# BananaFalls/LDPC-NeuralNetwork-Decoder

Measured on AMD Instinct MI355X. Metric: codewords/s at fixed SNR (BG2, 10 iters), higher is better.
Workload: dtype f32

## Files before the change

### ldpc-neuralnetwork-decoder_amd/csrc/flood.hip

```cpp
#include <algorithm>
#include <cstdio>
#include <cstdlib>
#include <string>
#include <vector>

#include "flood_host.hpp"

namespace ldpc {

__global__ void es_init_kernel(int32_t *ctl, uint64_t *staged, uint32_t *all_words) {
    const int t = threadIdx.x;
    if (t < 4) ctl[t] = 0;
    if (t < 4) staged[t] = 0;
    if (t < 64) all_words[t] = ~0u;
}

__global__ __launch_bounds__(1024) void counters_reduce_kernel(const uint32_t *__restrict__ partials, int64_t nwg,
                                                               uint64_t *counters, int32_t *batch_iters,
                                                               const int32_t *gate) {
    if (gate && *gate == 0) return;
    uint64_t acc[4] = {0, 0, 0, 0};
    uint32_t mx = 0;
    for (int64_t r = threadIdx.x; r < nwg; r += blockDim.x) {
        const uint32_t *row = partials + r * kPartRow;
// ... 63 lines not shown
        if (aw) {
            const int t = w * 32 + __builtin_ctz(aw);
            if (t < max_iter) { tstar = t; break; }
        }
    }
    const int wave = __builtin_amdgcn_readfirstlane(threadIdx.x >> 6);
    const Lane L = make_lane(T, nullptr, B);
    Ctx C;
    C.T = T;
    C.out_dtype = out_dtype;
    C.bits = bits;
    int errs = 0;
    emit_from_words(C, L, ws_words + ((int64_t)blockIdx.x * max_iter + tstar) * T.Nb, ~0ull, wave, errs);
    if (iters_out && L.valid && L.k == 0) iters_out[L.frame] = tstar + 1;
    const int nf = (int)min<int64_t>((int64_t)T.FG, B - (int64_t)blockIdx.x * T.FG);
    if (partials) reduce_counters(red, L, errs, tstar + 1, nf, T.Z, partials + (int64_t)blockIdx.x * kPartRow);
}

__global__ void fill_i32_kernel(int32_t *p, int32_t v) { *p = v; }

__global__ __launch_bounds__(256) void bp_math_kernel(const float *__restrict__ x, int64_t n,
                                                      float *__restrict__ th, float *__restrict__ at) {
    const int64_t i = (int64_t)blockIdx.x * blockDim.x + threadIdx.x;
    if (i >= n) return;
    const float v = x[i];
    if (th) th[i] = tanh_half(v);
    if (at) at[i] = two_atanh(v);
}

template <int ES>
__global__ __launch_bounds__(512) void flood_redo_kernel(FloodTables T, const float *__restrict__ llr, int64_t B,
// ... 71 lines not shown

bool has_redo(const ldpc_graph *g, int algo, int es) {
    return g->fixed_id != 0 && algo == LDPC_ALGO_MINSUM && (es == LDPC_ES_OFF || es == LDPC_ES_FRAME);
}

template <int ALGO, int ES>
int launch_flood(const ldpc_graph *g, const float *llr, int64_t B, int max_iter, float alpha, int out_dtype,
                 void *bits, const Outs &O, const EsWs &W, hipStream_t s, uint32_t *redo = nullptr) {
    const size_t lds = flood_lds_bytes(g, ES);
    const int64_t nwg = (B + g->FG - 1) / g->FG;
    if (g->fixed_id != 0) {
        const dim3 grid((unsigned)nwg), block(64 * g->ft.W);
        if constexpr (ALGO == LDPC_ALGO_MINSUM && (ES == LDPC_ES_OFF || ES == LDPC_ES_FRAME)) {
            if (redo) {
                LDPC_HIP(hipMemsetAsync(redo, 0, sizeof(uint32_t), s));
                int rc = launch_fixed_minsum(g->fixed_id, ES, grid, block, lds, s, g->ft, llr, B, max_iter, alpha,
                                             out_dtype, bits, O, W, redo);
                if (rc != LDPC_OK) return rc;
                auto again = flood_redo_kernel<ES>;
                LDPC_HIP(hipFuncSetAttribute(reinterpret_cast<const void *>(again),
                                             hipFuncAttributeMaxDynamicSharedMemorySize, (int)lds));
                Outs Or = O;
                Or.timeline = nullptr;
                hipLaunchKernelGGL(again, dim3((unsigned)std::min<int64_t>(nwg, kRedoGrid)), block, lds, s, g->ft, llr,
                                   B, max_iter, alpha, out_dtype, bits, Or, (const uint32_t *)redo);
                LDPC_CHECK_LAUNCH("flood_redo_kernel");
                return LDPC_OK;
            }
        }
        return ALGO == LDPC_ALGO_MINSUM
                   ? launch_fixed_minsum(g->fixed_id, ES, grid, block, lds, s, g->ft, llr, B, max_iter, alpha,
                                         out_dtype, bits, O, W, nullptr)
                   : launch_fixed_bp(g->fixed_id, ES, grid, block, lds, s, g->ft, llr, B, max_iter, alpha,
                                     out_dtype, bits, O, W);
    }
    auto kern = flood_kernel<ALGO, ES>;
    LDPC_HIP(hipFuncSetAttribute(reinterpret_cast<const void *>(kern),
                                 hipFuncAttributeMaxDynamicSharedMemorySize, (int)lds));
    hipLaunchKernelGGL(kern, dim3((unsigned)nwg), dim3(64 * g->ft.W), lds, s, g->ft, llr, B, max_iter, alpha,
                       out_dtype, bits, O, W);
    LDPC_CHECK_LAUNCH("flood_kernel");
    return LDPC_OK;
}

int reduce_rows(const ldpc_graph *g, int64_t B, const uint32_t *partials, uint64_t *counters, int32_t *batch_iters,
                const int32_t *gate, hipStream_t s, int frames_per_wg = 0) {
    if (!counters && !batch_iters) return LDPC_OK;
    const int fg = frames_per_wg > 0 ? frames_per_wg : g->FG;
// ... 182 lines not shown
```

### ldpc-neuralnetwork-decoder_amd/csrc/flood_dev.hpp

```cpp
#pragma once
#include <algorithm>
#include <cmath>
#include <cstdint>
#include <cstdlib>

#include <utility>

#include "common.hpp"
#include "gen/fixed_codes.hpp"
#include "graph.hpp"

namespace ldpc {

constexpr int kPartRow = 8;
constexpr int ES_P1 = 3, ES_P2 = 4;

struct EsWs {
    uint64_t *words;
    uint32_t *valid;
    int nvw;
    uint64_t *cand;
    int32_t *twg;
    int32_t *ctl;
    uint64_t *staged;
// ... 127 lines not shown
    if constexpr (DC % 2 == 0) p ^= __float_as_uint(v[DC - 1]);
    return p;
}

__device__ __forceinline__ float opaque_sf(float v) {
    asm volatile("" : "+s"(v));
    return v;
}
__device__ __forceinline__ uint32_t opaque_vu(uint32_t v) {
    asm volatile("" : "+v"(v));
    return v;
}
__device__ __forceinline__ float opaque_vf(float v) {
    asm volatile("" : "+v"(v));
    return v;
}
__device__ __forceinline__ void two_min_step(float &m1, float &m2, float x, float ninf) {
    m2 = __builtin_amdgcn_fmed3f(m1, fabsf(x), m2);
    m1 = __builtin_amdgcn_fmed3f(m1, fabsf(x), ninf);
}

__device__ __forceinline__ float vmin(float a, float b) { return __builtin_elementwise_minimum(a, b); }
__device__ __forceinline__ float vmax(float a, float b) { return __builtin_elementwise_maximum(a, b); }
template <int DC, int CAP>
__device__ __forceinline__ void two_smallest(const float (&v)[CAP], float &m1, float &m2, float ninf) {
    static_assert(DC <= CAP, "row longer than its buffer");
    if constexpr (DC == 1) {
        m1 = fabsf(v[0]);
    } else if constexpr (DC == 2) {
        m1 = vmin(fabsf(v[0]), fabsf(v[1]));
// ... 68 lines not shown
    const float big = __builtin_amdgcn_logf(r) * 0.693147180559945309f;
    return fabsf(x) < 0.5f ? small : big;
}

struct Ctx {
    FloodTables T;
    char *lds;
    uint64_t *words;
    uint32_t *flag;
    uint32_t *redo;
    float alpha;
    int out_dtype;
    void *bits;
    bool direct_bits;
    bool ballots;
};

__device__ __forceinline__ uint64_t seg_rotl(uint64_t w, int s, int z, uint64_t rep1) {
    if (s == 0) return w;
    if (z >= 64) return (w << s) | (w >> (64 - s));
    const uint64_t low = ((1ull << (z - s)) - 1ull) * rep1;
    return ((w & low) << s) | ((w & ~low) >> (z - s));
}

__device__ __forceinline__ void ext_decision(const Ctx &C, const Lane &L, int col, int s4, float app,
                                             int &errs) {
    const int bit = app < 0.0f;
    if (C.direct_bits && L.valid) {
        int64_t fr = L.frame;
        int k4 = L.k4;
// ... 233 lines not shown
}

__device__ __forceinline__ void emit_from_words(const Ctx &C, const Lane &L, const uint64_t *words, uint64_t mask,
                                                int wave, int &errs) {
    if (!(L.valid && ((mask >> L.f) & 1ull))) return;
    const int W1 = C.T.W + 1;
    for (int i = tab(C.T.prog_ptr, 3 * W1 + wave); i < tab(C.T.prog_ptr, 3 * W1 + wave + 1); ++i) {
        const int col = tab(C.T.bw_task, i);
        const int bit = (int)((words[col] >> L.lane) & 1ull);
        put_bit(C.bits, C.out_dtype, L.frame * C.T.N + (int64_t)col * L.Z() + L.k, bit);
        errs += bit;
    }
}

__device__ __forceinline__ void reduce_counters(void *lds, const Lane &L, int errs, int my_iters, int nf,
                                                int Z, uint32_t *row) {
    uint32_t *u = reinterpret_cast<uint32_t *>(lds);
    const int nt = blockDim.x;
    __syncthreads();
    u[threadIdx.x] = (uint32_t)errs;
    u[nt + threadIdx.x] = (uint32_t)my_iters;
    __syncthreads();
    if (threadIdx.x < 64) {
        const int f = threadIdx.x;
        uint32_t be = 0, fe = 0, fr = 0, it = 0, itmax = 0;
        if (f < nf) {
            for (int w = 0; w < nt / 64; ++w)
                for (int k = 0; k < Z; ++k) be += u[w * 64 + f * Z + k];
            fe = be > 0;
            fr = 1;
            it = u[nt + f * Z];
            itmax = it;
        }
        for (int off = 32; off > 0; off >>= 1) {
            be += __shfl_xor(be, off, 64);
            fe += __shfl_xor(fe, off, 64);
            fr += __shfl_xor(fr, off, 64);
            it += __shfl_xor(it, off, 64);
            itmax = max(itmax, (uint32_t)__shfl_xor(itmax, off, 64));
        }
        if (f == 0) {
            row[0] = be;
            row[1] = fe;
            row[2] = fr;
            row[3] = it;
            row[4] = itmax;
        }
    }
}

__device__ __forceinline__ Lane make_lane(const FloodTables &T, const float *llr, int64_t B, int group) {
    Lane L;
    L.group = group;
    L.lane = threadIdx.x & 63;
    const int lz = __builtin_ctz((unsigned)T.Z);
    L.f = L.lane >> lz;
    L.k = L.lane & (T.Z - 1);
    L.lane4 = 4 * L.lane;
    L.fz4 = 4 * (L.f << lz);
    L.k4 = 4 * L.k;
    L.z4 = 4 * T.Z;
    L.zmask4 = 4 * T.Z - 1;
    L.frame = (int64_t)group * T.FG + L.f;
    L.valid = L.frame < B;
    L.llr_row = reinterpret_cast<const char *>(llr ? llr + (L.valid ? L.frame : 0) * (int64_t)T.N : nullptr);
    return L;
}
__device__ __forceinline__ Lane make_lane(const FloodTables &T, const float *llr, int64_t B) {
    return make_lane(T, llr, B, (int)blockIdx.x);
}


#ifdef LDPC_EXP_NOBARRIER
#define LDPC_ITER_SYNC() ((void)0)
#else
#define LDPC_ITER_SYNC() __syncthreads()
#endif



template <int ES, class Body>
__device__ __forceinline__ void flood_drive(Body &body, Ctx &C, const Lane &L, int64_t B, int max_iter,
                                            const Outs &O, const EsWs &W) {
    const int tid = threadIdx.x;
    const int wave = __builtin_amdgcn_readfirstlane(tid >> 6);
    const int FG = C.T.FG, Nb = C.T.Nb, Z = C.T.Z;
    const int nf = (int)min<int64_t>((int64_t)FG, B - (int64_t)L.group * FG);
    const uint64_t exist = nf >= 64 ? ~0ull : ((1ull << nf) - 1ull);
    int errs = 0;
    if constexpr (ES == LDPC_ES_BATCH) {
        if (__builtin_amdgcn_readfirstlane(W.ctl[2]) == 0) return;
    }
    if constexpr (ES == ES_P2) {
        const int T = __builtin_amdgcn_readfirstlane(W.ctl[0]);
        if (__builtin_amdgcn_readfirstlane(W.twg[L.group]) == T) {
            emit_from_words(C, L, W.cand + (int64_t)L.group * Nb, exist, wave, errs);
            if (O.iters_out && L.valid && L.k == 0) O.iters_out[L.frame] = T;
            reduce_counters(C.lds, L, errs, T, nf, Z, O.partials + (int64_t)L.group * kPartRow);
            return;
        }
        max_iter = T;
    }
    if (tid == 0) *C.flag = 0;
    __syncthreads();
    body.init(C, L);
    __syncthreads();
#ifdef LDPC_TIMELINE
    uint64_t *tl = (O.timeline && blockIdx.x < (unsigned)kTlWgs && L.lane == 0)
                       ? O.timeline + ((int64_t)blockIdx.x * 4 + wave) * kTlPer : nullptr;
    auto mark = [&](int k) {
        uint64_t t;
        __builtin_amdgcn_sched_barrier(0);
        asm volatile("s_memtime %0\n\ts_waitcnt lgkmcnt(0)" : "=s"(t) : : "memory");
// ... 1 lines not shown
        if (tl && k < kTlPer - kTlTail) tl[k] = t;
    };
#else
    auto mark = [](int) {};
#endif
    mark(0);

    int my_iters = max_iter;
    uint64_t done = 0;
    constexpr bool kEvery = ES == LDPC_ES_BATCH || ES == LDPC_ES_FRAME || ES == ES_P1;
    for (int it = 0; it < max_iter; ++it) {
        const bool last = it == max_iter - 1;
        C.direct_bits = (ES == LDPC_ES_OFF || ES == ES_P2) && last;
        C.ballots = ES == LDPC_ES_BATCH || ES == LDPC_ES_FRAME || ES == ES_P1 || (ES == ES_P2 && last);
        if constexpr (Body::kBail) {
            if (__builtin_amdgcn_readfirstlane(*C.flag) != 0) {
                if (tid == 0) C.redo[1 + atomicAdd(C.redo, 1u)] = (uint32_t)L.group;
                return;
            }
        }
        if (kEvery || last)
            body.template check<true>(C, L, errs);
        else
            body.template check<false>(C, L, errs);
        mark(1 + 4 * it);
        LDPC_ITER_SYNC();
        mark(2 + 4 * it);
        if (C.ballots && tid == 0) C.words[Nb] = 0;
        if (last)
            body.template var<true, false>(C, L, errs);
        else if (kEvery)
            body.template var<true, true>(C, L, errs);
// ... 35 lines not shown
            } else if constexpr (ES == ES_P2) {
                if (vmask != exist && tid == 0) atomicOr(&W.ctl[1], 1);
            }
            __syncthreads();
            if (stop) break;
        }
    }
    if constexpr (ES == LDPC_ES_FRAME) {
        const uint64_t rest = exist & ~done;
        if (rest) {
            emit_from_words(C, L, C.words, rest, wave, errs);
            if (O.iters_out && L.valid && L.k == 0 && ((rest >> L.f) & 1ull)) O.iters_out[L.frame] = max_iter;
        }
    }
    if constexpr (ES == LDPC_ES_OFF || ES == ES_P2) {
        if (O.iters_out && L.valid && L.k == 0) O.iters_out[L.frame] = max_iter;
    }
    if constexpr (ES == LDPC_ES_OFF || ES == LDPC_ES_FRAME) {
        if (O.partials) reduce_counters(C.lds, L, errs, my_iters, nf, Z, O.partials + (int64_t)L.group * kPartRow);
    }
    if constexpr (ES == ES_P2) reduce_counters(C.lds, L, errs, max_iter, nf, Z, O.partials + (int64_t)L.group * kPartRow);
}

template <int ALGO>
struct GenericBody {
    static constexpr bool kBail = false;
    int wave;
    __device__ __forceinline__ void init(Ctx &C, const Lane &L) { init_phase(C, L, wave); }
    template <bool DEC>
    __device__ __forceinline__ void check(const Ctx &C, const Lane &L, int &errs) { check_phase<ALGO>(C, L, wave, errs); }
    template <bool DEC, bool WRITE>
    __device__ __forceinline__ void var(const Ctx &C, const Lane &L, int &errs) {
        var_phase(C, L, wave, WRITE, errs);
    }
    __device__ __forceinline__ int parity(const Ctx &C, const Lane &L) { return parity_phase(C, L, wave); }
};

__device__ __forceinline__ void init_ctx(Ctx &C, const FloodTables &T, char *lds, float alpha, int out_dtype,
                                         void *bits) {
    C.T = T;
    C.lds = lds;
    C.flag = reinterpret_cast<uint32_t *>(lds + (size_t)T.nslots * 256);
    C.words = reinterpret_cast<uint64_t *>(lds + (size_t)T.nslots * 256 + 8);
    C.alpha = alpha;
    C.out_dtype = out_dtype;
    C.bits = bits;
    C.direct_bits = false;
    C.ballots = false;
    C.redo = nullptr;
}

}

template <int ALGO, int ES>
__global__ __launch_bounds__(512) void flood_kernel(FloodTables T, const float *__restrict__ llr, int64_t B,
                                                    int max_iter, float alpha, int out_dtype,
                                                    void *__restrict__ bits, Outs O, EsWs W) {
    extern __shared__ __attribute__((aligned(16))) char lds[];
    const Lane L = make_lane(T, llr, B);
    Ctx C;
    init_ctx(C, T, lds, alpha, out_dtype, bits);
    GenericBody<ALGO> body{__builtin_amdgcn_readfirstlane((int)threadIdx.x >> 6)};
    flood_drive<ES>(body, C, L, B, max_iter, O, W);
}
// ... 17 lines not shown
#error "LDPC_REG_EDGES=1 needs the paired variable schedule (LDPC_VAR_PAIRS=1)"
#endif

#ifndef LDPC_SLOW_REG_EDGES
#define LDPC_SLOW_REG_EDGES 16
#endif
#ifndef LDPC_SLOW_REG_EDGES_OFF
#define LDPC_SLOW_REG_EDGES_OFF 6
#endif
constexpr int kAllRegEdges = 1 << 20;
template <int ES, bool BAIL>
constexpr int reg_edge_cap() {
    return BAIL ? kAllRegEdges : (ES == LDPC_ES_OFF ? LDPC_SLOW_REG_EDGES_OFF : LDPC_SLOW_REG_EDGES);
}

template <class G, int WV, int CAP>
struct FxPlan {
#if LDPC_REG_EDGES
    static constexpr int R0 = G::RE_CHK_PTR[WV], NR = G::RE_CHK_PTR[WV + 1] - R0;
    static constexpr int NREG = G::RE_NREG[WV] < CAP ? G::RE_NREG[WV] : CAP;
    static constexpr int chk_row(int i) { return G::RE_CHK_ROWS[R0 + i]; }
    static constexpr int row_shift(int e) { return G::RE_ROW_SHIFT[e]; }
    static constexpr int col_shift(int j) { return G::RE_COL_SHIFT[j]; }
    static constexpr int row_reg(int e) { return G::RE_ROW_REG[e] < CAP ? G::RE_ROW_REG[e] : -1; }
    static constexpr int col_reg(int j) { return G::RE_COL_REG[j] < CAP ? G::RE_COL_REG[j] : -1; }
#else
    static constexpr int R0 = G::CHK_PTR[WV], NR = G::CHK_PTR[WV + 1] - R0, NREG = 0;
    static constexpr int chk_row(int i) { return G::CHK_ROWS[R0 + i]; }
    static constexpr int row_shift(int e) { return G::ROW_SHIFT[e]; }
    static constexpr int col_shift(int j) { return G::COL_SHIFT[j]; }
    static constexpr int row_reg(int) { return -1; }
    static constexpr int col_reg(int) { return -1; }
// ... 79 lines not shown
        const float m = vmin(vmin(fabsf(v[A]), fabsf(v[B])), fabsf(v[Cc]));
        return __uint_as_float(__builtin_amdgcn_bitop3_b32(__float_as_uint(alv * m), xor3(bits(A), bits(B), bits(Cc)), sgn, 0x78));
    } else {
        constexpr int PE = E / 2;
        float m;
        if constexpr (DC == 5 && E == 4)
            m = vmin(pr[0], pr[1]);
        else if constexpr (DC == 5)
            m = vmin(vmin(fabsf(v[E ^ 1]), pr[1 - PE]), fabsf(v[4]));
        else
            m = vmin(vmin(fabsf(v[E ^ 1]), pr[(PE + 1) % 3]), pr[(PE + 2) % 3]);
        return __uint_as_float(__builtin_amdgcn_bitop3_b32(__float_as_uint(als * m), bits(E), sgn, 0x78));
    }
}

template <class G, int ALGO, int WV, bool BAIL, int CAP>
struct FixedBody {
    static_assert(!BAIL || ALGO == LDPC_ALGO_MINSUM, "only min-sum has a fast and an exact check update");
    static constexpr bool kBail = BAIL;
    using P = FxPlan<G, WV, CAP>;
    static constexpr int ZM4 = 4 * G::Z - 1;
    static constexpr int NEXT = P::T.next > 0 ? P::T.next : 1;
    static constexpr int NCOL = P::NC > 0 ? P::NC : 1;
    static constexpr int NSH = P::T.nsh > 0 ? P::T.nsh : 1;
    static constexpr int MAXDC = P::T.maxdc, MAXDV = P::T.maxdv;
    static constexpr int NRG = P::NREG > 0 ? P::NREG : 1;
    float ext[NEXT];
    float cllr[NCOL];
    uint32_t rot[NSH];
    float msg[NRG];

    __device__ __forceinline__ void init(Ctx &C, const Lane &L) {
        bool nan = false;
        sfor<P::NR>([&](auto i) {
            constexpr int I = decltype(i)::value, R = P::chk_row(I);
            constexpr int P0 = G::ROW_PTR[R], DC = G::ROW_PTR[R + 1] - P0;
            sfor<DC>([&](auto e) {
                constexpr int E = decltype(e)::value;
                if constexpr (G::ROW_SLOT[P0 + E] < 0) {
                    constexpr int X = P::ext_index(I, E), COL = G::ROW_COL[P0 + E], S4 = 4 * P::row_shift(P0 + E);
                    ext[X] = L.llr_at(COL * 4 * G::Z + ((L.k4 + S4) & ZM4));
                    nan |= !(fabsf(ext[X]) < INFINITY);
                }
            });
        });
        sfor<P::T.nsh>([&](auto j) {
            constexpr int J = decltype(j)::value, SH = P::T.shv[J];
// ... 2 lines not shown
                rot[J] = opaque_vu(base + L.lane4);
            else
                rot[J] = opaque_vu(base + L.fz4 + ((L.k4 + (4 * G::Z - 4 * SH)) & ZM4));
        });
        addtid_begin(C.lds);
        sfor<P::NC>([&](auto i) {
            constexpr int I = decltype(i)::value, COL = LDPC_VT(COLS)[P::C0 + I];
            constexpr int P0 = G::COL_PTR[COL], DV = G::COL_PTR[COL + 1] - P0;
            cllr[I] = L.llr_at(COL * 4 * G::Z + L.k4);
            nan |= !(fabsf(cllr[I]) < INFINITY);
            sfor<DV>([&](auto jj) {
                constexpr int J = P0 + decltype(jj)::value;
                if constexpr (P::col_reg(J) >= 0)
                    msg[P::col_reg(J)] = cllr[I];
                else
                    lds_wr_tid<G::COL_SLOT[J] * 256>(cllr[I]);
            });
        });
        addtid_end();
        if (__any(nan) && L.lane == 0) *C.flag = 1;
    }

    template <int I>
    __device__ __forceinline__ void load_row(const Ctx &C, const Lane &L, float (&v)[MAXDC]) const {
        constexpr int R = P::chk_row(I), P0 = G::ROW_PTR[R], DC = G::ROW_PTR[R + 1] - P0;
        sfor<DC>([&](auto e) {
            constexpr int E = decltype(e)::value, SL = G::ROW_SLOT[P0 + E];
            if constexpr (P::row_reg(P0 + E) >= 0)
                v[E] = msg[P::row_reg(P0 + E)];
            else if constexpr (SL >= 0)
                v[E] = lds_rd_abs<SL * 256>(rot[P::T.shidx[P::inv_shift(P::row_shift(P0 + E))]]);
            else
                v[E] = ext[P::ext_index(I, E)];
        });
    }

    template <int I, bool DEC, bool SLOW = false>
    __device__ __forceinline__ void row(const Ctx &C, const Lane &L, const float (&v)[MAXDC], int &errs, float ninf, float pinf, uint32_t sgn, float alv) {
        constexpr int R = P::chk_row(I), P0 = G::ROW_PTR[R], DC = G::ROW_PTR[R + 1] - P0;
        auto needed = [](int e) constexpr { return DEC || G::ROW_SLOT[P0 + e] >= 0; };
        auto emit = [&](auto e, float o) {
            constexpr int E = decltype(e)::value, SL = G::ROW_SLOT[P0 + E];
            if constexpr (P::row_reg(P0 + E) >= 0) {
                msg[P::row_reg(P0 + E)] = o;
            } else if constexpr (SL >= 0) {
                lds_wr_tid<SL * 256>(o);
            } else if constexpr (DEC) {
                if (C.direct_bits || C.ballots)
                    ext_decision(C, L, G::ROW_COL[P0 + E], 4 * P::row_shift(P0 + E), v[E] + o, errs);
            }
        };
        if constexpr (ALGO == LDPC_ALGO_MINSUM && !SLOW && DC >= 2 && DC <= kDirectDc) {
            float pr[3] = {};
            float als = alv;
            if constexpr (DC >= 5) {
                sfor<DC / 2>([&](auto j) {
                    constexpr int J = decltype(j)::value;
                    pr[J] = vmin(fabsf(v[2 * J]), fabsf(v[2 * J + 1]));
                });
                uint32_t par = xor3(__float_as_uint(v[0]), __float_as_uint(v[1]), __float_as_uint(v[2]));
                if constexpr (DC == 5)
                    par = xor3(par, __float_as_uint(v[3]), __float_as_uint(v[4]));
                else
                    par = xor3(par, __float_as_uint(v[3]), __float_as_uint(v[4])) ^ __float_as_uint(v[5]);
// ... 85 lines not shown
        static constexpr int NPREFA = HI == DA ? DA : (HI > 0 ? HI - 1 : 0);
        static constexpr bool BLAST = DB > 0 && LO <= DB - 1 && DB - 1 < HI;
        static constexpr int NPREF = NPREFA > (BLAST ? DB : 0) ? NPREFA : (BLAST ? DB : 0);
        static constexpr int NMSG = DA + DB;
    };
    struct TaskIn {
        f32x2 cp[MAXDV];
        float cs[MAXDV];
    };

    template <int X>
    __device__ __forceinline__ float c2v_in() const {
        if constexpr (P::col_reg(X) >= 0)
            return msg[P::col_reg(X)];
        else
            return lds_rd_abs<G::COL_SLOT[X] * 256>(rot[P::T.shidx[P::col_shift(X)]]);
    }
    template <int X>
    __device__ __forceinline__ void v2c_out(float o) {
        if constexpr (P::col_reg(X) >= 0)
            msg[P::col_reg(X)] = o;
        else
            lds_wr_tid<G::COL_SLOT[X] * 256>(o);
    }

    template <int TK>
    __device__ __forceinline__ void load_task(const Ctx &C, TaskIn &in) const {
        using K = Task<TK>;
        sfor<K::DA>([&](auto jj) {
            constexpr int J = decltype(jj)::value;
            if constexpr (J < K::DB) {
                in.cp[J].x = c2v_in<K::PA + J>();
                in.cp[J].y = c2v_in<K::PB + J>();
            } else {
                in.cs[J] = c2v_in<K::PA + J>();
            }
        });
    }
// ... 37 lines not shown
        });
        if constexpr (WRITE) {
            sfor<HI - LO>([&](auto q) {
                constexpr int E = LO + decltype(q)::value;
                if constexpr (E < DB) {
                    v2c_out<K::PA + E>(acc2[E].x);
                    v2c_out<K::PB + E>(acc2[E].y);
                } else {
                    v2c_out<K::PA + E>(accA[E]);
                }
            });
        }
        if constexpr (HI == DA) {
            if constexpr (ALGO == LDPC_ALGO_MINSUM) bad |= !(fabsf(PA) < INFINITY);
            if constexpr (DEC) {
                if (C.direct_bits || C.ballots) var_decision(C, L, K::CA, PA, errs);
            }
        }
        if constexpr (K::BLAST) {
            if constexpr (ALGO == LDPC_ALGO_MINSUM) bad |= !(fabsf(P2.y) < INFINITY);
            if constexpr (DEC) {
                if (C.direct_bits || C.ballots) var_decision(C, L, K::CB, P2.y, errs);
            }
        }
    }

    template <bool DEC, bool WRITE>
    __device__ __forceinline__ void var(const Ctx &C, const Lane &L, int &errs) {
        bool bad = false;
        if constexpr (P::NT > 0) {
            TaskIn ta, tb;
            if constexpr (WRITE) addtid_begin(C.lds);
            load_task<0>(C, ta);
            sfor<P::NT>([&](auto i) {
                constexpr int I = decltype(i)::value;
                constexpr bool more = I + 1 < P::NT;
                constexpr bool ahead = more && Task<I>::NMSG + Task<(more ? I + 1 : I)>::NMSG <= kVarPipe;
                if constexpr (I % 2 == 0) {
                    if constexpr (ahead) load_task<I + 1>(C, tb);
                    task<I, DEC, WRITE>(C, L, ta, errs, bad);
                    if constexpr (more && !ahead) load_task<(more ? I + 1 : I)>(C, tb);
                } else {
                    if constexpr (ahead) load_task<I + 1>(C, ta);
                    task<I, DEC, WRITE>(C, L, tb, errs, bad);
                    if constexpr (more && !ahead) load_task<(more ? I + 1 : I)>(C, ta);
                }
            });
            if constexpr (WRITE) addtid_end();
        }
        if constexpr (ALGO == LDPC_ALGO_MINSUM) {
            if (__any(bad) && L.lane == 0) *C.flag = 1;
        }
    }

    __device__ __forceinline__ int parity(const Ctx &C, const Lane &L) const {
        int inv = 0;
        int f = L.f, k = L.k;
        asm volatile("" : "+v"(f), "+v"(k));
        sfor<P::NR>([&](auto i) {
            constexpr int R = P::chk_row(decltype(i)::value);
            constexpr int P0 = G::ROW_PTR[R], DC = G::ROW_PTR[R + 1] - P0;
            int p = 0;
            sfor<DC>([&](auto e) {
                constexpr int E = decltype(e)::value;
                constexpr int COL = G::ROW_COL[P0 + E], S = P::row_shift(P0 + E);
                p ^= (int)(C.words[COL] >> (f * G::Z + ((k + S) & (G::Z - 1))));
// ... 3 lines not shown
        return inv & 1;
    }
};

template <class G, class F>
__device__ __forceinline__ void fx_by_wave(int wave, F &&f) {
    static_assert(G::W == 4, "fixed schedules are generated for 4 waves");
    switch (wave) {
        case 0: f(ic<0>{}); break;
        case 1: f(ic<1>{}); break;
        case 2: f(ic<2>{}); break;
        default: f(ic<3>{}); break;
    }
}

}

template <class G, int ALGO, int ES, bool BAIL = false>
__global__ __launch_bounds__(256, ES == LDPC_ES_OFF ? 4 : 3) void flood_fixed_kernel(FloodTables T, const float *__restrict__ llr,
                                                          int64_t B, int max_iter, float alpha, int out_dtype,
                                                          void *__restrict__ bits, Outs O, EsWs W, uint32_t *redo) {
    static_assert(!BAIL || ES == LDPC_ES_OFF || ES == LDPC_ES_FRAME, "the batch-stop passes share state across workgroups");
    extern __shared__ __attribute__((aligned(16))) char lds[];
#ifdef LDPC_TIMELINE
    const uint64_t t_in = tl_now();
#endif
    FloodTables Tc = T;
    Tc.Z = G::Z, Tc.FG = 64 / G::Z, Tc.Mb = G::Mb, Tc.Nb = G::Nb, Tc.N = G::N, Tc.nslots = G::NSLOTS, Tc.W = G::W;
    static_assert(G::Z < 64 && 64 % G::Z == 0, "rep1 below: a 1 at the bottom of every Z-bit segment");
    Tc.rep1 = ~0ull / ((1ull << G::Z) - 1ull);
    const Lane L = make_lane(Tc, llr, B);
    Ctx C;
    init_ctx(C, Tc, lds, alpha, out_dtype, bits);
    if constexpr (BAIL) C.redo = redo;
    fx_by_wave<G>(__builtin_amdgcn_readfirstlane((int)threadIdx.x >> 6), [&](auto wv) {
        FixedBody<G, ALGO, decltype(wv)::value, BAIL, reg_edge_cap<ES, BAIL>()> body;
        flood_drive<ES>(body, C, L, B, max_iter, O, W);
#ifdef LDPC_TIMELINE
        if constexpr (ES == LDPC_ES_OFF) tl_bracket(O.timeline, decltype(wv)::value, t_in);
#endif
    });
}

}
```

### ldpc-neuralnetwork-decoder_amd/csrc/flood_fixed_bp.hip

```cpp
#ifndef LDPC_REG_EDGES
#define LDPC_REG_EDGES 0
#endif
#include "flood_host.hpp"

namespace ldpc {

int launch_fixed_bp(int fixed_id, int es, dim3 grid, dim3 block, size_t lds, hipStream_t s,
                    const FloodTables &T, const float *llr, int64_t B, int max_iter, float alpha,
                    int out_dtype, void *bits, const Outs &O, const EsWs &W) {
    auto pick = [&](auto code) -> const void * {
        using G = decltype(code);
        switch (es) {
            case LDPC_ES_OFF: return reinterpret_cast<const void *>(flood_fixed_kernel<G, LDPC_ALGO_BP, LDPC_ES_OFF>);
            case LDPC_ES_FRAME: return reinterpret_cast<const void *>(flood_fixed_kernel<G, LDPC_ALGO_BP, LDPC_ES_FRAME>);
            case LDPC_ES_BATCH: return reinterpret_cast<const void *>(flood_fixed_kernel<G, LDPC_ALGO_BP, LDPC_ES_BATCH>);
            case ES_P1: return reinterpret_cast<const void *>(flood_fixed_kernel<G, LDPC_ALGO_BP, ES_P1>);
            case ES_P2: return reinterpret_cast<const void *>(flood_fixed_kernel<G, LDPC_ALGO_BP, ES_P2>);
            default: return nullptr;
        }
    };
    const void *kern = fixed_id == 1 ? pick(fixed::BG2_Z4{}) : (fixed_id == 2 ? pick(fixed::BG2_Z32{}) : nullptr);
    if (!kern) return fail(LDPC_EINVAL, "no fixed kernel for this code / stopping mode");
    LDPC_HIP(hipFuncSetAttribute(kern, hipFuncAttributeMaxDynamicSharedMemorySize, (int)lds));
    FloodTables t = T;
    const float *l = llr;
    int64_t b = B;
    int mi = max_iter;
    float a = alpha;
    int od = out_dtype;
    void *bi = bits;
    Outs o = O;
    EsWs w = W;
    uint32_t *rd = nullptr;
    void *args[] = {&t, &l, &b, &mi, &a, &od, &bi, &o, &w, &rd};
    LDPC_HIP(hipLaunchKernel(kern, grid, block, args, lds, s));
    return LDPC_OK;
// ... 4 lines not shown
```

### ldpc-neuralnetwork-decoder_amd/csrc/flood_fixed_ms.hip

```cpp
#include "flood_host.hpp"

namespace ldpc {

int launch_fixed_minsum(int fixed_id, int es, dim3 grid, dim3 block, size_t lds, hipStream_t s,
                        const FloodTables &T, const float *llr, int64_t B, int max_iter, float alpha,
                        int out_dtype, void *bits, const Outs &O, const EsWs &W, uint32_t *redo) {
    auto pick = [&](auto code) -> const void * {
        using G = decltype(code);
        if (redo && es == LDPC_ES_OFF) return reinterpret_cast<const void *>(flood_fixed_kernel<G, LDPC_ALGO_MINSUM, LDPC_ES_OFF, true>);
        if (redo && es == LDPC_ES_FRAME) return reinterpret_cast<const void *>(flood_fixed_kernel<G, LDPC_ALGO_MINSUM, LDPC_ES_FRAME, true>);
        if (redo) return nullptr;
        switch (es) {
            case LDPC_ES_OFF: return reinterpret_cast<const void *>(flood_fixed_kernel<G, LDPC_ALGO_MINSUM, LDPC_ES_OFF>);
            case LDPC_ES_FRAME: return reinterpret_cast<const void *>(flood_fixed_kernel<G, LDPC_ALGO_MINSUM, LDPC_ES_FRAME>);
            case LDPC_ES_BATCH: return reinterpret_cast<const void *>(flood_fixed_kernel<G, LDPC_ALGO_MINSUM, LDPC_ES_BATCH>);
            case ES_P1: return reinterpret_cast<const void *>(flood_fixed_kernel<G, LDPC_ALGO_MINSUM, ES_P1>);
            case ES_P2: return reinterpret_cast<const void *>(flood_fixed_kernel<G, LDPC_ALGO_MINSUM, ES_P2>);
            default: return nullptr;
        }
    };
    const void *kern = fixed_id == 1 ? pick(fixed::BG2_Z4{}) : (fixed_id == 2 ? pick(fixed::BG2_Z32{}) : nullptr);
    if (!kern) return fail(LDPC_EINVAL, "no fixed kernel for this code / stopping mode");
    LDPC_HIP(hipFuncSetAttribute(kern, hipFuncAttributeMaxDynamicSharedMemorySize, (int)lds));
    FloodTables t = T;
    const float *l = llr;
    int64_t b = B;
    int mi = max_iter;
    float a = alpha;
    int od = out_dtype;
    void *bi = bits;
    Outs o = O;
    EsWs w = W;
    uint32_t *rd = redo;
    void *args[] = {&t, &l, &b, &mi, &a, &od, &bi, &o, &w, &rd};
    LDPC_HIP(hipLaunchKernel(kern, grid, block, args, lds, s));
    return LDPC_OK;
// ... 4 lines not shown
```

### ldpc-neuralnetwork-decoder_amd/csrc/flood_host.hpp

```cpp
#pragma once
#include <cstddef>
#include <cstdint>

#include "flood_dev.hpp"

namespace ldpc {

constexpr int kStreamMaxDeg = 32;
inline size_t align256(size_t b) { return (b + 255) / 256 * 256; }

int reduce_counter_rows(const uint32_t *partials, int64_t nwg, uint64_t *counters, int32_t *batch_iters,
                        const int32_t *gate, hipStream_t s);

int launch_fixed_minsum(int fixed_id, int es, dim3 grid, dim3 block, size_t lds, hipStream_t s, const FloodTables &T,
                        const float *llr, int64_t B, int max_iter, float alpha, int out_dtype, void *bits,
                        const Outs &O, const EsWs &W, uint32_t *redo);
int launch_fixed_bp(int fixed_id, int es, dim3 grid, dim3 block, size_t lds, hipStream_t s, const FloodTables &T,
                    const float *llr, int64_t B, int max_iter, float alpha, int out_dtype, void *bits, const Outs &O,
                    const EsWs &W);

size_t layered_lds_bytes(const ldpc_graph *g, int es);
int run_layered(const ldpc_graph *g, const float *llr, int64_t B, int max_iter, float alpha, int es, int out_dtype,
                void *bits, int32_t *iters_out, uint64_t *counters, int32_t *batch_iters, void *work, hipStream_t s);

int64_t stream_ws_bytes(const ldpc_graph *g, int64_t B, int max_iter);
int run_stream_decode(int algo, const ldpc_graph *g, const float *llr, int64_t B, int max_iter, float alpha, int es,
                      int out_dtype, void *bits, int32_t *iters_out, uint64_t *counters, int32_t *batch_iters,
                      void *work, hipStream_t s);
int64_t custom_ws_bytes(const ldpc_graph *g, int64_t B);
int run_custom_minsum(const ldpc_graph *g, const float *llr, int64_t B, int iterations, float *probs, void *work,
                      hipStream_t s);

// ... 2 lines not shown
```

Measured before the change: 70.70 million.

## Compact LDS slots to spilled edges only and raise bail-kernel occupancy

LDS slots for edge messages are renumbered so that only edges not held in registers take shared memory, and each fixed kernel instantiation gets its own computed LDS size instead of the generic host value. The bail (redo) min-sum kernel now targets 4 workgroups per CU. It also recomputes lane and thread identity from hardware lane intrinsics and uniform wave indices so those values need not stay live across the decode loop. The aim is lower LDS and register pressure so more workgroups can be resident. The cost is more kernel template complexity, and tighter launch bounds could force register spills.

```diff
diff --git a/ldpc-neuralnetwork-decoder_amd/csrc/flood.hip b/ldpc-neuralnetwork-decoder_amd/csrc/flood.hip
--- a/ldpc-neuralnetwork-decoder_amd/csrc/flood.hip
+++ b/ldpc-neuralnetwork-decoder_amd/csrc/flood.hip
@@ -101,7 +101,7 @@
     emit_from_words(C, L, ws_words + ((int64_t)blockIdx.x * max_iter + tstar) * T.Nb, ~0ull, wave, errs);
     if (iters_out && L.valid && L.k == 0) iters_out[L.frame] = tstar + 1;
     const int nf = (int)min<int64_t>((int64_t)T.FG, B - (int64_t)blockIdx.x * T.FG);
-    if (partials) reduce_counters(red, L, errs, tstar + 1, nf, T.Z, partials + (int64_t)blockIdx.x * kPartRow);
+    if (partials) reduce_counters(red, L, errs, tstar + 1, nf, T.Z, partials + (int64_t)blockIdx.x * kPartRow, (int)threadIdx.x);
 }
 
 __global__ void fill_i32_kernel(int32_t *p, int32_t v) { *p = v; }
@@ -203,7 +203,7 @@
         if constexpr (ALGO == LDPC_ALGO_MINSUM && (ES == LDPC_ES_OFF || ES == LDPC_ES_FRAME)) {
             if (redo) {
                 LDPC_HIP(hipMemsetAsync(redo, 0, sizeof(uint32_t), s));
-                int rc = launch_fixed_minsum(g->fixed_id, ES, grid, block, lds, s, g->ft, llr, B, max_iter, alpha,
+                int rc = launch_fixed_minsum(g->fixed_id, ES, grid, block, s, g->ft, llr, B, max_iter, alpha,
                                              out_dtype, bits, O, W, redo);
                 if (rc != LDPC_OK) return rc;
                 auto again = flood_redo_kernel<ES>;
@@ -218,9 +218,9 @@
             }
         }
         return ALGO == LDPC_ALGO_MINSUM
-                   ? launch_fixed_minsum(g->fixed_id, ES, grid, block, lds, s, g->ft, llr, B, max_iter, alpha,
+                   ? launch_fixed_minsum(g->fixed_id, ES, grid, block, s, g->ft, llr, B, max_iter, alpha,
                                          out_dtype, bits, O, W, nullptr)
-                   : launch_fixed_bp(g->fixed_id, ES, grid, block, lds, s, g->ft, llr, B, max_iter, alpha,
+                   : launch_fixed_bp(g->fixed_id, ES, grid, block, s, g->ft, llr, B, max_iter, alpha,
                                      out_dtype, bits, O, W);
     }
     auto kern = flood_kernel<ALGO, ES>;
diff --git a/ldpc-neuralnetwork-decoder_amd/csrc/flood_dev.hpp b/ldpc-neuralnetwork-decoder_amd/csrc/flood_dev.hpp
--- a/ldpc-neuralnetwork-decoder_amd/csrc/flood_dev.hpp
+++ b/ldpc-neuralnetwork-decoder_amd/csrc/flood_dev.hpp
@@ -165,6 +165,11 @@
 __device__ __forceinline__ float opaque_vf(float v) {
     asm volatile("" : "+v"(v));
     return v;
+}
+__device__ __forceinline__ int hw_lane() {
+    uint32_t lane;
+    asm volatile("v_mbcnt_lo_u32_b32 %0, -1, 0\n\tv_mbcnt_hi_u32_b32 %0, -1, %0" : "=v"(lane));
+    return (int)lane;
 }
 __device__ __forceinline__ void two_min_step(float &m1, float &m2, float x, float ninf) {
     m2 = __builtin_amdgcn_fmed3f(m1, fabsf(x), m2);
@@ -263,6 +268,8 @@
     void *bits;
     bool direct_bits;
     bool ballots;
+    const float *llr;
+    int64_t B;
 };
 
 __device__ __forceinline__ uint64_t seg_rotl(uint64_t w, int s, int z, uint64_t rep1) {
@@ -526,15 +533,15 @@
 }
 
 __device__ __forceinline__ void reduce_counters(void *lds, const Lane &L, int errs, int my_iters, int nf,
-                                                int Z, uint32_t *row) {
+                                                int Z, uint32_t *row, int tid) {
     uint32_t *u = reinterpret_cast<uint32_t *>(lds);
     const int nt = blockDim.x;
     __syncthreads();
-    u[threadIdx.x] = (uint32_t)errs;
-    u[nt + threadIdx.x] = (uint32_t)my_iters;
+    u[tid] = (uint32_t)errs;
+    u[nt + tid] = (uint32_t)my_iters;
     __syncthreads();
-    if (threadIdx.x < 64) {
-        const int f = threadIdx.x;
+    if (tid < 64) {
+        const int f = tid;
         uint32_t be = 0, fe = 0, fr = 0, it = 0, itmax = 0;
         if (f < nf) {
             for (int w = 0; w < nt / 64; ++w)
@@ -561,10 +568,10 @@
     }
 }
 
-__device__ __forceinline__ Lane make_lane(const FloodTables &T, const float *llr, int64_t B, int group) {
+__device__ __forceinline__ Lane make_lane(const FloodTables &T, const float *llr, int64_t B, int group, int lane) {
     Lane L;
     L.group = group;
-    L.lane = threadIdx.x & 63;
+    L.lane = lane;
     const int lz = __builtin_ctz((unsigned)T.Z);
     L.f = L.lane >> lz;
     L.k = L.lane & (T.Z - 1);
@@ -578,6 +585,9 @@
     L.llr_row = reinterpret_cast<const char *>(llr ? llr + (L.valid ? L.frame : 0) * (int64_t)T.N : nullptr);
     return L;
 }
+__device__ __forceinline__ Lane make_lane(const FloodTables &T, const float *llr, int64_t B, int group) {
+    return make_lane(T, llr, B, group, (int)(threadIdx.x & 63));
+}
 __device__ __forceinline__ Lane make_lane(const FloodTables &T, const float *llr, int64_t B) {
     return make_lane(T, llr, B, (int)blockIdx.x);
 }
@@ -594,8 +604,8 @@
 template <int ES, class Body>
 __device__ __forceinline__ void flood_drive(Body &body, Ctx &C, const Lane &L, int64_t B, int max_iter,
                                             const Outs &O, const EsWs &W) {
-    const int tid = threadIdx.x;
-    const int wave = __builtin_amdgcn_readfirstlane(tid >> 6);
+    const int tid = body.tid();
+    const int wave = body.wave_index();
     const int FG = C.T.FG, Nb = C.T.Nb, Z = C.T.Z;
     const int nf = (int)min<int64_t>((int64_t)FG, B - (int64_t)L.group * FG);
     const uint64_t exist = nf >= 64 ? ~0ull : ((1ull << nf) - 1ull);
@@ -608,7 +618,7 @@
         if (__builtin_amdgcn_readfirstlane(W.twg[L.group]) == T) {
             emit_from_words(C, L, W.cand + (int64_t)L.group * Nb, exist, wave, errs);
             if (O.iters_out && L.valid && L.k == 0) O.iters_out[L.frame] = T;
-            reduce_counters(C.lds, L, errs, T, nf, Z, O.partials + (int64_t)L.group * kPartRow);
+            reduce_counters(C.lds, L, errs, T, nf, Z, O.partials + (int64_t)L.group * kPartRow, tid);
             return;
         }
         max_iter = T;
@@ -640,8 +650,11 @@
         C.direct_bits = (ES == LDPC_ES_OFF || ES == ES_P2) && last;
         C.ballots = ES == LDPC_ES_BATCH || ES == LDPC_ES_FRAME || ES == ES_P1 || (ES == ES_P2 && last);
         if constexpr (Body::kBail) {
+            if (!kEvery && last) errs = 0;
             if (__builtin_amdgcn_readfirstlane(*C.flag) != 0) {
-                if (tid == 0) C.redo[1 + atomicAdd(C.redo, 1u)] = (uint32_t)L.group;
+                uint32_t grp = (uint32_t)L.group;
+                asm volatile("" : "+s"(grp));
+                if (wave == 0 && hw_lane() == 0) C.redo[1 + atomicAdd(C.redo, 1u)] = grp;
                 return;
             }
         }
@@ -707,12 +720,17 @@
         }
     }
     if constexpr (ES == LDPC_ES_OFF || ES == ES_P2) {
-        if (O.iters_out && L.valid && L.k == 0) O.iters_out[L.frame] = max_iter;
+        if (O.iters_out) {
+            const Lane Le = body.lane(C, L);
+            if (Le.valid && Le.k == 0) O.iters_out[Le.frame] = max_iter;
+        }
     }
     if constexpr (ES == LDPC_ES_OFF || ES == LDPC_ES_FRAME) {
-        if (O.partials) reduce_counters(C.lds, L, errs, my_iters, nf, Z, O.partials + (int64_t)L.group * kPartRow);
-    }
-    if constexpr (ES == ES_P2) reduce_counters(C.lds, L, errs, max_iter, nf, Z, O.partials + (int64_t)L.group * kPartRow);
+        if (O.partials)
+            reduce_counters(C.lds, L, errs, my_iters, nf, Z, O.partials + (int64_t)L.group * kPartRow,
+                            Body::kBail ? wave * 64 + hw_lane() : tid);
+    }
+    if constexpr (ES == ES_P2) reduce_counters(C.lds, L, errs, max_iter, nf, Z, O.partials + (int64_t)L.group * kPartRow, tid);
 }
 
 template <int ALGO>
@@ -720,6 +738,9 @@
     static constexpr bool kBail = false;
     int wave;
     __device__ __forceinline__ void init(Ctx &C, const Lane &L) { init_phase(C, L, wave); }
+    __device__ __forceinline__ const Lane &lane(const Ctx &, const Lane &L) const { return L; }
+    __device__ __forceinline__ int tid() const { return threadIdx.x; }
+    __device__ __forceinline__ int wave_index() const { return wave; }
     template <bool DEC>
     __device__ __forceinline__ void check(const Ctx &C, const Lane &L, int &errs) { check_phase<ALGO>(C, L, wave, errs); }
     template <bool DEC, bool WRITE>
@@ -741,6 +762,12 @@
     C.direct_bits = false;
     C.ballots = false;
     C.redo = nullptr;
+    C.llr = nullptr;
+    C.B = 0;
+}
+
+__device__ __forceinline__ Lane fresh_lane(const Ctx &C, int group) {
+    return make_lane(C.T, C.llr, C.B, group, hw_lane());
 }
 
 }
@@ -788,8 +815,33 @@
     return BAIL ? kAllRegEdges : (ES == LDPC_ES_OFF ? LDPC_SLOW_REG_EDGES_OFF : LDPC_SLOW_REG_EDGES);
 }
 
+template <class G, int CAP>
+struct FxSlots {
+    struct Tab {
+        int n = 0;
+        int at[G::NSLOTS] = {};
+    };
+    static constexpr Tab make() {
+        Tab t{};
+        for (int e = 0; e < G::NBLOCKS; ++e) {
+            if (G::ROW_SLOT[e] < 0) continue;
+#if LDPC_REG_EDGES
+            const bool reg = G::RE_ROW_REG[e] >= 0 && G::RE_ROW_REG[e] < CAP;
+#else
+            const bool reg = false;
+#endif
+            t.at[G::ROW_SLOT[e]] = reg ? -1 : t.n++;
+        }
+        return t;
+    }
+    static constexpr Tab T = make();
+    static constexpr int N = T.n;
+};
+
 template <class G, int WV, int CAP>
 struct FxPlan {
+    static constexpr int row_slot(int e) { return FxSlots<G, CAP>::T.at[G::ROW_SLOT[e]]; }
+    static constexpr int col_slot(int j) { return FxSlots<G, CAP>::T.at[G::COL_SLOT[j]]; }
 #if LDPC_REG_EDGES
     static constexpr int R0 = G::RE_CHK_PTR[WV], NR = G::RE_CHK_PTR[WV + 1] - R0;
     static constexpr int NREG = G::RE_NREG[WV] < CAP ? G::RE_NREG[WV] : CAP;
@@ -899,7 +951,7 @@
     }
 }
 
-template <class G, int ALGO, int WV, bool BAIL, int CAP>
+template <class G, int ALGO, int WV, bool BAIL, int CAP, int PIPE = kVarPipe, bool RELANE = false>
 struct FixedBody {
     static_assert(!BAIL || ALGO == LDPC_ALGO_MINSUM, "only min-sum has a fast and an exact check update");
     static constexpr bool kBail = BAIL;
@@ -915,7 +967,15 @@
     uint32_t rot[NSH];
     float msg[NRG];
 
-    __device__ __forceinline__ void init(Ctx &C, const Lane &L) {
+    __device__ __forceinline__ Lane lane(const Ctx &C, const Lane &L) const { return BAIL ? fresh_lane(C, L.group) : L; }
+    __device__ __forceinline__ Lane dec_lane(const Ctx &C, const Lane &L) const { return RELANE ? fresh_lane(C, L.group) : L; }
+    __device__ __forceinline__ int tid() const { return BAIL ? WV * 64 + hw_lane() : (int)threadIdx.x; }
+    __device__ __forceinline__ int wave_index() const {
+        return BAIL ? WV : __builtin_amdgcn_readfirstlane((int)threadIdx.x >> 6);
+    }
+
+    __device__ __forceinline__ void init(Ctx &C, const Lane &L0) {
+        const Lane L = lane(C, L0);
         bool nan = false;
         sfor<P::NR>([&](auto i) {
             constexpr int I = decltype(i)::value, R = P::chk_row(I);
@@ -948,7 +1008,7 @@
                 if constexpr (P::col_reg(J) >= 0)
                     msg[P::col_reg(J)] = cllr[I];
                 else
-                    lds_wr_tid<G::COL_SLOT[J] * 256>(cllr[I]);
+                    lds_wr_tid<P::col_slot(J) * 256>(cllr[I]);
             });
         });
         addtid_end();
@@ -963,7 +1023,7 @@
             if constexpr (P::row_reg(P0 + E) >= 0)
                 v[E] = msg[P::row_reg(P0 + E)];
             else if constexpr (SL >= 0)
-                v[E] = lds_rd_abs<SL * 256>(rot[P::T.shidx[P::inv_shift(P::row_shift(P0 + E))]]);
+                v[E] = lds_rd_abs<P::row_slot(P0 + E) * 256>(rot[P::T.shidx[P::inv_shift(P::row_shift(P0 + E))]]);
             else
                 v[E] = ext[P::ext_index(I, E)];
         });
@@ -978,10 +1038,10 @@
             if constexpr (P::row_reg(P0 + E) >= 0) {
                 msg[P::row_reg(P0 + E)] = o;
             } else if constexpr (SL >= 0) {
-                lds_wr_tid<SL * 256>(o);
+                lds_wr_tid<P::row_slot(P0 + E) * 256>(o);
             } else if constexpr (DEC) {
                 if (C.direct_bits || C.ballots)
-                    ext_decision(C, L, G::ROW_COL[P0 + E], 4 * P::row_shift(P0 + E), v[E] + o, errs);
+                    ext_decision(C, dec_lane(C, L), G::ROW_COL[P0 + E], 4 * P::row_shift(P0 + E), v[E] + o, errs);
             }
         };
         if constexpr (ALGO == LDPC_ALGO_MINSUM && !SLOW && DC >= 2 && DC <= kDirectDc) {
@@ -1097,14 +1157,14 @@
         if constexpr (P::col_reg(X) >= 0)
             return msg[P::col_reg(X)];
         else
-            return lds_rd_abs<G::COL_SLOT[X] * 256>(rot[P::T.shidx[P::col_shift(X)]]);
+            return lds_rd_abs<P::col_slot(X) * 256>(rot[P::T.shidx[P::col_shift(X)]]);
     }
     template <int X>
     __device__ __forceinline__ void v2c_out(float o) {
         if constexpr (P::col_reg(X) >= 0)
             msg[P::col_reg(X)] = o;
         else
-            lds_wr_tid<G::COL_SLOT[X] * 256>(o);
+            lds_wr_tid<P::col_slot(X) * 256>(o);
     }
 
     template <int TK>
@@ -1172,13 +1232,13 @@
         if constexpr (HI == DA) {
             if constexpr (ALGO == LDPC_ALGO_MINSUM) bad |= !(fabsf(PA) < INFINITY);
             if constexpr (DEC) {
-                if (C.direct_bits || C.ballots) var_decision(C, L, K::CA, PA, errs);
+                if (C.direct_bits || C.ballots) var_decision(C, dec_lane(C, L), K::CA, PA, errs);
             }
         }
         if constexpr (K::BLAST) {
             if constexpr (ALGO == LDPC_ALGO_MINSUM) bad |= !(fabsf(P2.y) < INFINITY);
             if constexpr (DEC) {
-                if (C.direct_bits || C.ballots) var_decision(C, L, K::CB, P2.y, errs);
+                if (C.direct_bits || C.ballots) var_decision(C, dec_lane(C, L), K::CB, P2.y, errs);
             }
         }
     }
@@ -1193,7 +1253,7 @@
             sfor<P::NT>([&](auto i) {
                 constexpr int I = decltype(i)::value;
                 constexpr bool more = I + 1 < P::NT;
-                constexpr bool ahead = more && Task<I>::NMSG + Task<(more ? I + 1 : I)>::NMSG <= kVarPipe;
+                constexpr bool ahead = more && Task<I>::NMSG + Task<(more ? I + 1 : I)>::NMSG <= PIPE;
                 if constexpr (I % 2 == 0) {
                     if constexpr (ahead) load_task<I + 1>(C, tb);
                     task<I, DEC, WRITE>(C, L, ta, errs, bad);
@@ -1207,7 +1267,7 @@
             if constexpr (WRITE) addtid_end();
         }
         if constexpr (ALGO == LDPC_ALGO_MINSUM) {
-            if (__any(bad) && L.lane == 0) *C.flag = 1;
+            if (__any(bad) && (BAIL || L.lane == 0)) *C.flag = 1;
         }
     }
 
@@ -1241,10 +1301,26 @@
     }
 }
 
+template <class G, int ES, bool BAIL>
+constexpr int fixed_nslots() {
+    return FxSlots<G, reg_edge_cap<ES, BAIL>()>::N;
+}
+template <class G, int ES, bool BAIL>
+constexpr size_t fixed_lds_bytes() {
+    const size_t b = (size_t)fixed_nslots<G, ES, BAIL>() * 256 + 8 + (ES != LDPC_ES_OFF ? (size_t)(G::Nb + 1) * 8 : 0);
+    const size_t red = 2 * 64 * (size_t)G::W * sizeof(uint32_t);
+    return b > red ? b : red;
+}
+
+template <int ES, bool BAIL>
+constexpr int fixed_wgs_per_cu() {
+    return ES == LDPC_ES_OFF || BAIL ? 4 : 3;
+}
+
 }
 
 template <class G, int ALGO, int ES, bool BAIL = false>
-__global__ __launch_bounds__(256, ES == LDPC_ES_OFF ? 4 : 3) void flood_fixed_kernel(FloodTables T, const float *__restrict__ llr,
+__global__ __launch_bounds__(256, (fixed_wgs_per_cu<ES, BAIL>())) void flood_fixed_kernel(FloodTables T, const float *__restrict__ llr,
                                                           int64_t B, int max_iter, float alpha, int out_dtype,
                                                           void *__restrict__ bits, Outs O, EsWs W, uint32_t *redo) {
     static_assert(!BAIL || ES == LDPC_ES_OFF || ES == LDPC_ES_FRAME, "the batch-stop passes share state across workgroups");
@@ -1253,15 +1329,18 @@
     const uint64_t t_in = tl_now();
 #endif
     FloodTables Tc = T;
-    Tc.Z = G::Z, Tc.FG = 64 / G::Z, Tc.Mb = G::Mb, Tc.Nb = G::Nb, Tc.N = G::N, Tc.nslots = G::NSLOTS, Tc.W = G::W;
+    Tc.Z = G::Z, Tc.FG = 64 / G::Z, Tc.Mb = G::Mb, Tc.Nb = G::Nb, Tc.N = G::N, Tc.nslots = fixed_nslots<G, ES, BAIL>(), Tc.W = G::W;
     static_assert(G::Z < 64 && 64 % G::Z == 0, "rep1 below: a 1 at the bottom of every Z-bit segment");
     Tc.rep1 = ~0ull / ((1ull << G::Z) - 1ull);
     const Lane L = make_lane(Tc, llr, B);
     Ctx C;
     init_ctx(C, Tc, lds, alpha, out_dtype, bits);
     if constexpr (BAIL) C.redo = redo;
-    fx_by_wave<G>(__builtin_amdgcn_readfirstlane((int)threadIdx.x >> 6), [&](auto wv) {
-        FixedBody<G, ALGO, decltype(wv)::value, BAIL, reg_edge_cap<ES, BAIL>()> body;
+    C.llr = llr, C.B = B;
+    int wave = __builtin_amdgcn_readfirstlane((int)threadIdx.x >> 6);
+    if constexpr (BAIL) asm volatile("" : "+s"(wave));
+    fx_by_wave<G>(wave, [&](auto wv) {
+        FixedBody<G, ALGO, decltype(wv)::value, BAIL, reg_edge_cap<ES, BAIL>(), kVarPipe, BAIL && ES == LDPC_ES_OFF> body;
         flood_drive<ES>(body, C, L, B, max_iter, O, W);
 #ifdef LDPC_TIMELINE
         if constexpr (ES == LDPC_ES_OFF) tl_bracket(O.timeline, decltype(wv)::value, t_in);
diff --git a/ldpc-neuralnetwork-decoder_amd/csrc/flood_fixed_bp.hip b/ldpc-neuralnetwork-decoder_amd/csrc/flood_fixed_bp.hip
--- a/ldpc-neuralnetwork-decoder_amd/csrc/flood_fixed_bp.hip
+++ b/ldpc-neuralnetwork-decoder_amd/csrc/flood_fixed_bp.hip
@@ -5,21 +5,34 @@
 
 namespace ldpc {
 
-int launch_fixed_bp(int fixed_id, int es, dim3 grid, dim3 block, size_t lds, hipStream_t s,
+int launch_fixed_bp(int fixed_id, int es, dim3 grid, dim3 block, hipStream_t s,
                     const FloodTables &T, const float *llr, int64_t B, int max_iter, float alpha,
                     int out_dtype, void *bits, const Outs &O, const EsWs &W) {
-    auto pick = [&](auto code) -> const void * {
+    struct Inst {
+        const void *kern;
+        size_t lds;
+    };
+    auto pick = [&](auto code) -> Inst {
         using G = decltype(code);
+        auto inst = [](auto es_c, auto bail_c) -> Inst {
+            constexpr int ES = decltype(es_c)::value;
+            constexpr bool BAIL = decltype(bail_c)::value;
+            return {reinterpret_cast<const void *>(flood_fixed_kernel<G, LDPC_ALGO_BP, ES, BAIL>),
+                    fixed_lds_bytes<G, ES, BAIL>()};
+        };
+        using std::false_type;
         switch (es) {
-            case LDPC_ES_OFF: return reinterpret_cast<const void *>(flood_fixed_kernel<G, LDPC_ALGO_BP, LDPC_ES_OFF>);
-            case LDPC_ES_FRAME: return reinterpret_cast<const void *>(flood_fixed_kernel<G, LDPC_ALGO_BP, LDPC_ES_FRAME>);
-            case LDPC_ES_BATCH: return reinterpret_cast<const void *>(flood_fixed_kernel<G, LDPC_ALGO_BP, LDPC_ES_BATCH>);
-            case ES_P1: return reinterpret_cast<const void *>(flood_fixed_kernel<G, LDPC_ALGO_BP, ES_P1>);
-            case ES_P2: return reinterpret_cast<const void *>(flood_fixed_kernel<G, LDPC_ALGO_BP, ES_P2>);
-            default: return nullptr;
+            case LDPC_ES_OFF: return inst(ic<LDPC_ES_OFF>{}, false_type{});
+            case LDPC_ES_FRAME: return inst(ic<LDPC_ES_FRAME>{}, false_type{});
+            case LDPC_ES_BATCH: return inst(ic<LDPC_ES_BATCH>{}, false_type{});
+            case ES_P1: return inst(ic<ES_P1>{}, false_type{});
+            case ES_P2: return inst(ic<ES_P2>{}, false_type{});
+            default: return Inst{nullptr, 0};
         }
     };
-    const void *kern = fixed_id == 1 ? pick(fixed::BG2_Z4{}) : (fixed_id == 2 ? pick(fixed::BG2_Z32{}) : nullptr);
+    const Inst in = fixed_id == 1 ? pick(fixed::BG2_Z4{}) : (fixed_id == 2 ? pick(fixed::BG2_Z32{}) : Inst{nullptr, 0});
+    const void *kern = in.kern;
+    const size_t lds = in.lds;
     if (!kern) return fail(LDPC_EINVAL, "no fixed kernel for this code / stopping mode");
     LDPC_HIP(hipFuncSetAttribute(kern, hipFuncAttributeMaxDynamicSharedMemorySize, (int)lds));
     FloodTables t = T;
diff --git a/ldpc-neuralnetwork-decoder_amd/csrc/flood_fixed_ms.hip b/ldpc-neuralnetwork-decoder_amd/csrc/flood_fixed_ms.hip
--- a/ldpc-neuralnetwork-decoder_amd/csrc/flood_fixed_ms.hip
+++ b/ldpc-neuralnetwork-decoder_amd/csrc/flood_fixed_ms.hip
@@ -2,24 +2,38 @@
 
 namespace ldpc {
 
-int launch_fixed_minsum(int fixed_id, int es, dim3 grid, dim3 block, size_t lds, hipStream_t s,
+int launch_fixed_minsum(int fixed_id, int es, dim3 grid, dim3 block, hipStream_t s,
                         const FloodTables &T, const float *llr, int64_t B, int max_iter, float alpha,
                         int out_dtype, void *bits, const Outs &O, const EsWs &W, uint32_t *redo) {
-    auto pick = [&](auto code) -> const void * {
+    struct Inst {
+        const void *kern;
+        size_t lds;
+    };
+    auto pick = [&](auto code) -> Inst {
         using G = decltype(code);
-        if (redo && es == LDPC_ES_OFF) return reinterpret_cast<const void *>(flood_fixed_kernel<G, LDPC_ALGO_MINSUM, LDPC_ES_OFF, true>);
-        if (redo && es == LDPC_ES_FRAME) return reinterpret_cast<const void *>(flood_fixed_kernel<G, LDPC_ALGO_MINSUM, LDPC_ES_FRAME, true>);
-        if (redo) return nullptr;
+        auto inst = [](auto es_c, auto bail_c) -> Inst {
+            constexpr int ES = decltype(es_c)::value;
+            constexpr bool BAIL = decltype(bail_c)::value;
+            return {reinterpret_cast<const void *>(flood_fixed_kernel<G, LDPC_ALGO_MINSUM, ES, BAIL>),
+                    fixed_lds_bytes<G, ES, BAIL>()};
+        };
+        using std::false_type;
+        using std::true_type;
+        if (redo && es == LDPC_ES_OFF) return inst(ic<LDPC_ES_OFF>{}, true_type{});
+        if (redo && es == LDPC_ES_FRAME) return inst(ic<LDPC_ES_FRAME>{}, true_type{});
+        if (redo) return Inst{nullptr, 0};
         switch (es) {
-            case LDPC_ES_OFF: return reinterpret_cast<const void *>(flood_fixed_kernel<G, LDPC_ALGO_MINSUM, LDPC_ES_OFF>);
-            case LDPC_ES_FRAME: return reinterpret_cast<const void *>(flood_fixed_kernel<G, LDPC_ALGO_MINSUM, LDPC_ES_FRAME>);
-            case LDPC_ES_BATCH: return reinterpret_cast<const void *>(flood_fixed_kernel<G, LDPC_ALGO_MINSUM, LDPC_ES_BATCH>);
-            case ES_P1: return reinterpret_cast<const void *>(flood_fixed_kernel<G, LDPC_ALGO_MINSUM, ES_P1>);
-            case ES_P2: return reinterpret_cast<const void *>(flood_fixed_kernel<G, LDPC_ALGO_MINSUM, ES_P2>);
-            default: return nullptr;
+            case LDPC_ES_OFF: return inst(ic<LDPC_ES_OFF>{}, false_type{});
+            case LDPC_ES_FRAME: return inst(ic<LDPC_ES_FRAME>{}, false_type{});
+            case LDPC_ES_BATCH: return inst(ic<LDPC_ES_BATCH>{}, false_type{});
+            case ES_P1: return inst(ic<ES_P1>{}, false_type{});
+            case ES_P2: return inst(ic<ES_P2>{}, false_type{});
+            default: return Inst{nullptr, 0};
         }
     };
-    const void *kern = fixed_id == 1 ? pick(fixed::BG2_Z4{}) : (fixed_id == 2 ? pick(fixed::BG2_Z32{}) : nullptr);
+    const Inst in = fixed_id == 1 ? pick(fixed::BG2_Z4{}) : (fixed_id == 2 ? pick(fixed::BG2_Z32{}) : Inst{nullptr, 0});
+    const void *kern = in.kern;
+    const size_t lds = in.lds;
     if (!kern) return fail(LDPC_EINVAL, "no fixed kernel for this code / stopping mode");
     LDPC_HIP(hipFuncSetAttribute(kern, hipFuncAttributeMaxDynamicSharedMemorySize, (int)lds));
     FloodTables t = T;
diff --git a/ldpc-neuralnetwork-decoder_amd/csrc/flood_host.hpp b/ldpc-neuralnetwork-decoder_amd/csrc/flood_host.hpp
--- a/ldpc-neuralnetwork-decoder_amd/csrc/flood_host.hpp
+++ b/ldpc-neuralnetwork-decoder_amd/csrc/flood_host.hpp
@@ -12,10 +12,10 @@
 int reduce_counter_rows(const uint32_t *partials, int64_t nwg, uint64_t *counters, int32_t *batch_iters,
                         const int32_t *gate, hipStream_t s);
 
-int launch_fixed_minsum(int fixed_id, int es, dim3 grid, dim3 block, size_t lds, hipStream_t s, const FloodTables &T,
+int launch_fixed_minsum(int fixed_id, int es, dim3 grid, dim3 block, hipStream_t s, const FloodTables &T,
                         const float *llr, int64_t B, int max_iter, float alpha, int out_dtype, void *bits,
                         const Outs &O, const EsWs &W, uint32_t *redo);
-int launch_fixed_bp(int fixed_id, int es, dim3 grid, dim3 block, size_t lds, hipStream_t s, const FloodTables &T,
+int launch_fixed_bp(int fixed_id, int es, dim3 grid, dim3 block, hipStream_t s, const FloodTables &T,
                     const float *llr, int64_t B, int max_iter, float alpha, int out_dtype, void *bits, const Outs &O,
                     const EsWs &W);
 
```

After: 70.33 million. Within noise of the previous version (-0.5%).
